# codex-storage/nim-groth16

Measured on AMD Instinct MI355X. Metric: proofs/sec (BN254 Groth16, 2^20-constraint circuit), higher is better.
Workload: dtype u32 (254-bit Montgomery: 8x32-bit limbs; 9x29-bit limbs in the bucket accumulation); 1 GPU; BN254 2^20-constraint synthetic R1CS (squaring chain, m=2^20-2), full prove: buildABC + 6 NTT + 4 G1 MSM + 1 G2 MSM, snarkjs flavour, 1 proof/step/GPU (3 proofs in flight per GPU, one shared key); mode=replica, nvars=1048576, domain_log2=20

## Files before the change

### nim_groth16_amd/csrc/msm.cuh

```cuda
#pragma once
#include "ec29.cuh"
#include "msm_params.hpp"

namespace g16 {

#ifndef G16_ACC_BLOCK
#define G16_ACC_BLOCK 256
#endif
constexpr int ACC_BLOCK = G16_ACC_BLOCK;
#ifndef G16_G2_WAVES
#define G16_G2_WAVES 2
#endif

#ifndef G16_TAIL_PRIO
#define G16_TAIL_PRIO 0
#endif
__device__ __forceinline__ void tail_prio() {
#if G16_TAIL_PRIO
  __builtin_amdgcn_s_setprio(G16_TAIL_PRIO);
#endif
}
#ifndef G16_G1_WAVES
#define G16_G1_WAVES 4
#endif
#ifndef G16_TAIL_WAVES_G1
#define G16_TAIL_WAVES_G1 1
#endif
#ifndef G16_TAIL_WAVES_G2
#define G16_TAIL_WAVES_G2 1
#endif
template <class C>
constexpr int tail_waves() { return sizeof(typename C::Aff) == 64 ? G16_TAIL_WAVES_G1 : G16_TAIL_WAVES_G2; }

constexpr int MSM_BATCH_MAX = 3;
template <class C>
struct MsmJob {
  const typename Ec29<C>::Tab* points;
  const uint32_t* entries;
  const uint32_t* offset;
  const uint2* xseg;
  const uint32_t* info;
  const uint32_t* perm;
  const uint32_t* heavy;
  const uint32_t* xoff;
  typename Ec29<C>::Acc* partial;
  const typename Ec29<C>::Acc* init;
  typename C::Acc* chunkR;
  typename C::Acc* chunkA;
  typename C::Acc* wsum;
  typename C::Aff* out_aff;
  typename C::Acc* out_acc;
};
template <class C>
struct MsmBatch {
  MsmJob<C> job[MSM_BATCH_MAX];
};



template <class EMIT>
__device__ __forceinline__ void msm_digits(const u256* __restrict__ scalars, const uint32_t* __restrict__ live, uint32_t i,
                                           const MsmParams& P, EMIT&& emit) {
  if (live && !((live[i >> 5] >> (i & 31)) & 1u)) return;
  u256 s = scalars[i];
  if (P.scalars_mont) s = Fr::from_mont(s);
  if (Fr::is_zero(s)) return;
  const uint32_t c = P.c, half = 1u << (c - 1), mask = (1u << c) - 1;
  uint32_t carry = 0;
  for (uint32_t w = 0; w < P.nwin; ++w) {
    uint32_t raw = (s.v[0] & mask) + carry;
    uint32_t neg = raw > half ? 1u : 0u;
    uint32_t mag = neg ? (1u << c) - raw : raw;
    carry = neg;
    if (mag) {
      if (P.mtab == 2) {
        uint32_t sel;
        const uint32_t b = msm_class_bucket(mag, c, sel);
        emit(w + sel * P.nwin, b, neg);
      } else {
        emit(w, mag - 1, neg);
      }
    }
#pragma unroll
    for (int j = 0; j < 7; ++j) s.v[j] = __builtin_amdgcn_alignbit(s.v[j + 1], s.v[j], c);
    s.v[7] >>= c;
  }
}

template <bool LEAN>
__device__ __forceinline__ void msm_entry_place(const MsmParams& P, uint32_t w, uint32_t i, uint32_t shift,
                                                uint32_t& set_off, uint32_t& pidx) {
  if (LEAN) {
    uint32_t table, set;
    msm_window_slot(w, P.tstride, table, set);
    set_off = set << shift;
    pidx = table * P.n + i;
  } else {
    set_off = P.tables ? 0u : (w << shift);
    pidx = P.tables ? (w * P.n + i) : i;
  }
}

template <bool LEAN>
static __global__ void __launch_bounds__(MSM_BLOCK) msm_count(const u256* __restrict__ scalars,
                                                              const uint32_t* __restrict__ live, MsmParams P,
                                                              uint32_t* __restrict__ count) {
  uint32_t i = blockIdx.x * MSM_BLOCK + threadIdx.x;
  if (i >= P.n) return;
  const uint32_t bshift = P.c - 1;
  msm_digits(scalars, live, i, P, [&](uint32_t w, uint32_t k, uint32_t) {
    uint32_t set_off, pidx;
    msm_entry_place<LEAN>(P, w, i, bshift, set_off, pidx);
    atomicAdd(&count[set_off + k], 1u);
  });
}

template <bool LEAN>
static __global__ void __launch_bounds__(MSM_BLOCK) msm_scatter(const u256* __restrict__ scalars,
                                                         const uint32_t* __restrict__ live, MsmParams P,
                                                         const uint32_t* __restrict__ offset,
                                                         uint32_t* __restrict__ cursor,
                                                         uint32_t* __restrict__ entries) {
  uint32_t i = blockIdx.x * MSM_BLOCK + threadIdx.x;
  if (i >= P.n) return;
  const uint32_t bshift = P.c - 1;
  msm_digits(scalars, live, i, P, [&](uint32_t w, uint32_t k, uint32_t neg) {
    uint32_t set_off, pidx;
    msm_entry_place<LEAN>(P, w, i, bshift, set_off, pidx);
    uint32_t b = set_off + k;
    uint32_t pos = offset[b] + atomicAdd(&cursor[b], 1u);
    entries[pos] = pidx | (neg << 31);
  });
}

__device__ __forceinline__ uint32_t lds_rank_add(uint32_t* ctr, uint32_t key) {
  const uint32_t leader = __builtin_amdgcn_readfirstlane(key);
  const unsigned long long m = __ballot(key == leader);
  if (__popcll(m) > 8) {
    uint32_t r = 0;
    if (key == leader) {
      const uint32_t lane = threadIdx.x & 63;
      const uint32_t before = __popcll(m & ((1ull << lane) - 1));
      uint32_t base = 0;
      if (before == 0) base = atomicAdd(&ctr[leader], (uint32_t)__popcll(m));
      base = __shfl(base, __ffsll((long long)m) - 1, 64);
      r = base + before;
    } else {
      r = atomicAdd(&ctr[key], 1u);
    }
    return r;
  }
  return atomicAdd(&ctr[key], 1u);
}

__device__ __forceinline__ uint32_t part_tile_of_block(uint32_t bid, uint32_t ntiles) {
  return (ntiles & 7u) ? bid : (bid & 7u) * (ntiles >> 3) + (bid >> 3);
}
template <bool SCATTER, bool LEAN>
static __global__ void __launch_bounds__(PART_BLOCK) part_pass(const u256* __restrict__ scalars,
                                                               const uint32_t* __restrict__ live, MsmParams P,
                                                               uint32_t lo_bits, uint32_t nparts, uint32_t ntiles,
                                                               uint32_t* __restrict__ tile_hist,
                                                               uint2* __restrict__ tmp) {
  __shared__ uint32_t hist[PART_MAX];
  const uint32_t tile = part_tile_of_block(blockIdx.x, ntiles);
  for (uint32_t p = threadIdx.x; p < nparts; p += PART_BLOCK)
    hist[p] = SCATTER ? tile_hist[(size_t)p * ntiles + tile] : 0u;
  __syncthreads();
  const uint32_t hi_bits = P.c - 1 - lo_bits, lo_mask = (1u << lo_bits) - 1;
  for (uint32_t r = 0; r < PART_PER_THREAD; ++r) {
    uint32_t i = tile * PART_TILE + r * PART_BLOCK + threadIdx.x;
    if (i < P.n) {
      msm_digits(scalars, live, i, P, [&](uint32_t w, uint32_t k, uint32_t neg) {
        uint32_t set_off, pidx;
        msm_entry_place<LEAN>(P, w, i, hi_bits, set_off, pidx);
        uint32_t part = set_off | (k >> lo_bits);
        uint32_t pos = lds_rank_add(hist, part);
        if (SCATTER) tmp[pos] = make_uint2((k & lo_mask) | (neg << BS_LOG), pidx);
      });
    }
  }
  if (!SCATTER) {
    __syncthreads();
    for (uint32_t p = threadIdx.x; p < nparts; p += PART_BLOCK) tile_hist[(size_t)p * ntiles + tile] = hist[p];
  }
}

__device__ __forceinline__ void bs_slice(uint32_t start, uint32_t end, uint32_t q, uint32_t& lo, uint32_t& hi) {
  const uint32_t len = end - start;
  lo = start + (uint32_t)(((uint64_t)len * q) / BS_SPLIT);
  hi = start + (uint32_t)(((uint64_t)len * (q + 1)) / BS_SPLIT);
}
static __global__ void __launch_bounds__(BS_LOW) bucket_hist(const uint2* __restrict__ tmp,
                                                          const uint32_t* __restrict__ part_base, uint32_t ntiles,
                                                          uint32_t nparts, const uint32_t* __restrict__ total,
                                                          uint32_t* __restrict__ slice_hist) {
  __shared__ uint32_t hist[BS_LOW];
  uint32_t part, q;
  bs_block(blockIdx.x, nparts, part, q);
  const uint32_t tid = threadIdx.x;
  const uint32_t start = part_base[(size_t)part * ntiles];
  const uint32_t end = part + 1 < nparts ? part_base[(size_t)(part + 1) * ntiles] : total[0];
  uint32_t lo, hi;
  bs_slice(start, end, q, lo, hi);
  hist[tid] = 0;
  __syncthreads();
  for (uint32_t j = lo + tid; j < hi; j += BS_LOW) lds_rank_add(hist, tmp[j].x & (uint32_t)(BS_LOW - 1));
  __syncthreads();
  slice_hist[((size_t)part * BS_SPLIT + q) * BS_LOW + tid] = hist[tid];
}
__device__ __forceinline__ uint32_t extra_segs(uint32_t cnt, uint32_t L) { return cnt > L ? (cnt - 1) / L : 0u; }
static __global__ void __launch_bounds__(BS_LOW) bucket_place(const uint2* __restrict__ tmp,
                                                           const uint32_t* __restrict__ part_base, uint32_t ntiles,
                                                           uint32_t nparts, const uint32_t* __restrict__ total,
                                                           const uint32_t* __restrict__ slice_hist, MsmParams P,
                                                           uint32_t lo_bits, uint32_t* __restrict__ count,
                                                           uint32_t* __restrict__ offset,
                                                           uint32_t* __restrict__ entries, uint32_t fused,
                                                           uint32_t* __restrict__ xoff, uint32_t* __restrict__ heavy,
                                                           uint32_t* __restrict__ info, uint32_t* __restrict__ ghist,
                                                           uint32_t* __restrict__ blk_base) {
  __shared__ uint32_t cur[BS_LOW];
  __shared__ uint32_t szh[PERM_BINS];
  uint32_t part, q;
  bs_block(blockIdx.x, nparts, part, q);
  const uint32_t tid = threadIdx.x;
  const uint32_t start = part_base[(size_t)part * ntiles];
  const uint32_t end = part + 1 < nparts ? part_base[(size_t)(part + 1) * ntiles] : total[0];
  uint32_t mine = 0, before = 0;
#pragma unroll
  for (int k = 0; k < BS_SPLIT; ++k) {
    uint32_t h = slice_hist[((size_t)part * BS_SPLIT + k) * BS_LOW + tid];
    mine += h;
    if ((uint32_t)k < q) before += h;
  }
  cur[tid] = mine;
  if (tid < PERM_BINS) szh[tid] = 0;
  __syncthreads();
  for (int d = 1; d < BS_LOW; d <<= 1) {
    uint32_t add = (int)tid >= d ? cur[tid - d] : 0u;
    __syncthreads();
    cur[tid] += add;
    __syncthreads();
  }
  const uint32_t excl = cur[tid] - mine;
  __syncthreads();
  cur[tid] = start + excl + before;
  if (q == 0) {
    if (tid < (1u << lo_bits)) {
      uint32_t b = (part << lo_bits) + tid;
      count[b] = mine;
      offset[b] = start + excl;
      if (fused) {
        const uint32_t e = extra_segs(mine, P.seg);
        uint32_t x0 = 0;
        if (e) {
          x0 = atomicAdd(&info[1], e);
          heavy[atomicAdd(&info[2], 1u)] = b;
        }
        xoff[b] = x0;
        atomicAdd(&szh[mine < PERM_BINS - 1 ? mine : PERM_BINS - 1], 1u);
      }
    }
    if (part == nparts - 1 && tid == 0) offset[P.nbuckets] = end;
  }
  __syncthreads();
  if (q == 0 && fused && tid < PERM_BINS) {
    const uint32_t m = szh[tid];
    blk_base[(size_t)part * PERM_BINS + tid] = m ? atomicAdd(&ghist[tid], m) : 0u;
  }
  uint32_t lo, hi;
  bs_slice(start, end, q, lo, hi);
  for (uint32_t j = lo + tid; j < hi; j += BS_LOW) {
    uint2 e = tmp[j];
    uint32_t pos = lds_rank_add(cur, e.x & (uint32_t)(BS_LOW - 1));
    entries[pos] = e.y | (((e.x >> BS_LOG) & 1u) << 31);
  }
}


constexpr uint32_t HEAVY_MIN = 12;

__device__ __forceinline__ uint2 block_excl_scan2(uint2 v, uint2* total) {
  __shared__ uint2 wsum[SCAN_BLOCK / 64];
  const uint32_t lane = threadIdx.x & 63, wave = threadIdx.x >> 6;
  uint2 inc = v;
#pragma unroll
  for (int d = 1; d < 64; d <<= 1) {
    uint32_t x = __shfl_up(inc.x, d, 64), y = __shfl_up(inc.y, d, 64);
    if (lane >= (uint32_t)d) { inc.x += x; inc.y += y; }
  }
  if (lane == 63) wsum[wave] = inc;
  __syncthreads();
  uint2 base = make_uint2(0, 0), tot = make_uint2(0, 0);
#pragma unroll
  for (int w = 0; w < SCAN_BLOCK / 64; ++w) {
    uint2 s = wsum[w];
    if ((uint32_t)w < wave) { base.x += s.x; base.y += s.y; }
    tot.x += s.x; tot.y += s.y;
  }
  __syncthreads();
  if (total) *total = tot;
  return make_uint2(base.x + inc.x - v.x, base.y + inc.y - v.y);
}

static __global__ void __launch_bounds__(SCAN_BLOCK) scan_tile_sums(const uint32_t* __restrict__ count, uint32_t nb,
                                                             uint32_t L, uint2* __restrict__ tile_sum) {
  uint32_t base = blockIdx.x * SCAN_TILE + threadIdx.x * SCAN_ITEMS;
  uint2 s = make_uint2(0, 0);
#pragma unroll
  for (int j = 0; j < SCAN_ITEMS; ++j) {
    uint32_t b = base + j;
    uint32_t cnt = b < nb ? count[b] : 0u;
    s.x += cnt;
    s.y += extra_segs(cnt, L);
  }
  uint2 tot;
  block_excl_scan2(s, &tot);
  if (threadIdx.x == 0) tile_sum[blockIdx.x] = tot;
}
static __global__ void __launch_bounds__(SCAN_BLOCK) scan_tiles(uint2* __restrict__ tile_sum, uint32_t ntiles,
                                                         uint32_t* __restrict__ info) {
  uint2 carry = make_uint2(0, 0);
  for (uint32_t base = 0; base < ntiles; base += SCAN_BLOCK) {
    uint32_t t = base + threadIdx.x;
    uint2 v = t < ntiles ? tile_sum[t] : make_uint2(0, 0);
    uint2 tot;
    uint2 ex = block_excl_scan2(v, &tot);
    if (t < ntiles) tile_sum[t] = make_uint2(ex.x + carry.x, ex.y + carry.y);
    carry.x += tot.x;
    carry.y += tot.y;
  }
  if (threadIdx.x == 0) {
    info[0] = carry.x;
    info[1] = carry.y;
  }
}
static __global__ void __launch_bounds__(SCAN_BLOCK) scan_apply(const uint32_t* __restrict__ count, uint32_t nb, uint32_t L,
                                                         const uint2* __restrict__ tile_sum,
                                                         uint32_t* __restrict__ offset, uint32_t* __restrict__ xoff,
                                                         uint32_t* __restrict__ heavy, uint32_t* __restrict__ info) {
  uint32_t base = blockIdx.x * SCAN_TILE + threadIdx.x * SCAN_ITEMS;
  uint32_t cnt[SCAN_ITEMS];
  uint2 s = make_uint2(0, 0);
#pragma unroll
  for (int j = 0; j < SCAN_ITEMS; ++j) {
    uint32_t b = base + j;
    cnt[j] = b < nb ? count[b] : 0u;
    s.x += cnt[j];
    s.y += extra_segs(cnt[j], L);
  }
  uint2 ex = block_excl_scan2(s, nullptr);
  uint2 t0 = tile_sum[blockIdx.x];
  uint32_t o = t0.x + ex.x, x = t0.y + ex.y;
#pragma unroll
  for (int j = 0; j < SCAN_ITEMS; ++j) {
    uint32_t b = base + j;
    if (b < nb) {
      offset[b] = o;
      xoff[b] = x;
      uint32_t e = extra_segs(cnt[j], L);
      if (e) heavy[atomicAdd(&info[2], 1u)] = b;
      o += cnt[j];
      x += e;
    }
  }
  if (blockIdx.x == gridDim.x - 1 && threadIdx.x == SCAN_BLOCK - 1) offset[nb] = o;
}

static __global__ void __launch_bounds__(SCAN_BLOCK) scan1_tile_sums(const uint32_t* __restrict__ v, uint32_t n,
                                                                     uint2* __restrict__ tile_sum) {
  uint32_t base = blockIdx.x * SCAN_TILE + threadIdx.x * SCAN_ITEMS;
  uint2 s = make_uint2(0, 0);
#pragma unroll
  for (int j = 0; j < SCAN_ITEMS; ++j) s.x += base + j < n ? v[base + j] : 0u;
  uint2 tot;
  block_excl_scan2(s, &tot);
  if (threadIdx.x == 0) tile_sum[blockIdx.x] = tot;
}
static __global__ void __launch_bounds__(SCAN_BLOCK) scan1_apply(uint32_t* __restrict__ v, uint32_t n,
                                                                 const uint2* __restrict__ tile_sum) {
  uint32_t base = blockIdx.x * SCAN_TILE + threadIdx.x * SCAN_ITEMS;
  uint32_t x[SCAN_ITEMS];
  uint2 s = make_uint2(0, 0);
#pragma unroll
  for (int j = 0; j < SCAN_ITEMS; ++j) {
    x[j] = base + j < n ? v[base + j] : 0u;
    s.x += x[j];
  }
  uint2 ex = block_excl_scan2(s, nullptr);
  uint32_t o = tile_sum[blockIdx.x].x + ex.x;
#pragma unroll
  for (int j = 0; j < SCAN_ITEMS; ++j) {
    if (base + j < n) v[base + j] = o;
    o += x[j];
  }
}

static __global__ void __launch_bounds__(MSM_BLOCK) msm_make_extra(const uint32_t* __restrict__ heavy,
                                                            const uint32_t* __restrict__ info,
                                                            const uint32_t* __restrict__ offset,
                                                            const uint32_t* __restrict__ xoff, uint32_t L,
                                                            uint32_t max_extra, uint2* __restrict__ xseg) {
  const uint32_t nheavy = info[2];
  for (uint32_t h = blockIdx.x; h < nheavy; h += gridDim.x) {
    uint32_t b = heavy[h];
    uint32_t cnt = offset[b + 1] - offset[b];
    uint32_t e = extra_segs(cnt, L), x0 = xoff[b];
    for (uint32_t s = threadIdx.x; s < e; s += MSM_BLOCK)
      if (x0 + s < max_extra) xseg[x0 + s] = make_uint2(b, s + 1);
  }
}

static __global__ void __launch_bounds__(PERM_BLOCK) perm_hist(const uint32_t* __restrict__ count, uint32_t nb,
                                                               uint32_t* __restrict__ ghist,
                                                               uint32_t* __restrict__ blk_base) {
  __shared__ uint32_t h[PERM_BINS];
  if (threadIdx.x < PERM_BINS) h[threadIdx.x] = 0;
  __syncthreads();
  uint32_t b = blockIdx.x * PERM_BLOCK + threadIdx.x;
  if (b < nb) {
    uint32_t c = count[b];
    atomicAdd(&h[c < PERM_BINS - 1 ? c : PERM_BINS - 1], 1u);
  }
  __syncthreads();
  if (threadIdx.x < PERM_BINS) {
    uint32_t mine = h[threadIdx.x];
    blk_base[(size_t)blockIdx.x * PERM_BINS + threadIdx.x] = mine ? atomicAdd(&ghist[threadIdx.x], mine) : 0u;
  }
}
static __global__ void __launch_bounds__(PERM_BLOCK) perm_scatter(const uint32_t* __restrict__ count, uint32_t nb,
                                                                  const uint32_t* __restrict__ ghist,
                                                                  const uint32_t* __restrict__ blk_base,
                                                                  uint32_t* __restrict__ perm) {
  __shared__ uint32_t start[PERM_BINS];
  __shared__ uint32_t cur[PERM_BINS];
  const bool bin = threadIdx.x < PERM_BINS;
  if (bin) {
    start[threadIdx.x] = ghist[threadIdx.x];
    cur[threadIdx.x] = 0;
  }
  __syncthreads();
  for (int d = 1; d < PERM_BINS; d <<= 1) {
    uint32_t add = bin && (int)threadIdx.x + d < PERM_BINS ? start[threadIdx.x + d] : 0u;
    __syncthreads();
    if (bin) start[threadIdx.x] += add;
    __syncthreads();
  }
  uint32_t incl = bin ? start[threadIdx.x] : 0u;
  __syncthreads();
  if (bin) start[threadIdx.x] = incl - ghist[threadIdx.x];
  __syncthreads();
  uint32_t b = blockIdx.x * PERM_BLOCK + threadIdx.x;
  if (b < nb) {
    uint32_t c = count[b];
    uint32_t v = c < PERM_BINS - 1 ? c : PERM_BINS - 1;
    uint32_t r = atomicAdd(&cur[v], 1u);
    perm[start[v] + blk_base[(size_t)blockIdx.x * PERM_BINS + v] + r] = b;
  }
}

template <class C>
__global__ void __launch_bounds__(ACC_BLOCK, sizeof(typename C::Aff) == 64 ? G16_G1_WAVES : G16_G2_WAVES)
msm_accum(const MsmBatch<C> B, MsmParams P, unsigned long long* __restrict__ clk) {
  using E = Ec29<C>;
  const MsmJob<C>& J = B.job[blockIdx.y];
  const typename E::Tab* __restrict__ points = J.points;
  const uint32_t* __restrict__ entries = J.entries;
  const uint32_t* __restrict__ offset = J.offset;
  unsigned long long t0 = 0, r0 = 0;
  const bool stamp = clk != nullptr && threadIdx.x == 0;
  if (stamp) t0 = __builtin_amdgcn_s_memtime(), r0 = __builtin_amdgcn_s_memrealtime();
  const uint32_t t = blockIdx.x * ACC_BLOCK + threadIdx.x;
  const uint32_t nx = J.info[1] < P.max_extra ? J.info[1] : P.max_extra;
  uint32_t b, s, slot;
  if (t < nx) {
    uint2 d = J.xseg[t];
    b = d.x;
    s = d.y;
    slot = P.nbuckets + t;
  } else {
    if (t - nx >= P.nbuckets) return;
    b = J.perm[t - nx];
    s = 0;
    slot = b;
  }
  uint32_t beg = offset[b], end = offset[b + 1];
  beg += s * P.seg;
  if (end > beg + P.seg) end = beg + P.seg;
  typename E::Acc acc = E::acc_inf();
  if (J.init != nullptr && s == 0) acc = J.init[b];
  for (uint32_t j = beg; j < end; ++j) {
    const uint32_t e = entries[j];
    E::madd(acc, points + (e & 0x7fffffffu), e >> 31);
  }
  J.partial[slot] = acc;
  if (stamp) {
    atomicAdd(&clk[0], __builtin_amdgcn_s_memtime() - t0);
    atomicAdd(&clk[1], __builtin_amdgcn_s_memrealtime() - r0);
  }
}

template <class C>
__global__ void __launch_bounds__(MSM_BLOCK) points_to29(const typename C::Aff* __restrict__ points, uint32_t n,
                                                         typename Ec29<C>::Tab* __restrict__ out) {
  uint32_t i = blockIdx.x * MSM_BLOCK + threadIdx.x;
  if (i < n) out[i] = Ec29<C>::tab_from_std(points[i]);
}

template <class C, int BLOCK>
__device__ __forceinline__ typename C::Acc block_sum(typename C::Acc v, typename C::Acc* sh) {
  sh[threadIdx.x] = v;
  __syncthreads();
#pragma unroll 1
  for (int stride = BLOCK / 2; stride > 0; stride >>= 1) {
    if ((int)threadIdx.x < stride) {
      typename C::Acc a = sh[threadIdx.x];
      C::add(a, sh[threadIdx.x + stride]);
      sh[threadIdx.x] = a;
    }
    __syncthreads();
  }
  typename C::Acc r = sh[0];
  __syncthreads();
  return r;
}

template <class C>
constexpr int heavy_block() { return sizeof(typename C::Aff) == 64 ? 256 : 128; }
template <class C>
__global__ void __launch_bounds__(heavy_block<C>(), tail_waves<C>()) msm_heavy(const MsmBatch<C> B, MsmParams P) {
  tail_prio();
  using E = Ec29<C>;
  constexpr int HEAVY_BLOCK = heavy_block<C>();
  extern __shared__ __align__(16) unsigned char smem[];
  typename E::Acc* sh = reinterpret_cast<typename E::Acc*>(smem);
  const MsmJob<C>& J = B.job[blockIdx.y];
  const uint32_t* __restrict__ heavy = J.heavy;
  const uint32_t* __restrict__ offset = J.offset;
  const uint32_t* __restrict__ xoff = J.xoff;
  typename E::Acc* __restrict__ partial = J.partial;
  const uint32_t nheavy = J.info[2];
  for (uint32_t h = blockIdx.x * HEAVY_BLOCK + threadIdx.x; h < nheavy; h += gridDim.x * HEAVY_BLOCK) {
    const uint32_t b = heavy[h];
    const uint32_t e = extra_segs(offset[b + 1] - offset[b], P.seg), x0 = xoff[b];
    if (e >= HEAVY_MIN) continue;
    typename E::Acc acc = partial[b];
    for (uint32_t k = 0; k < e; ++k) E::add(acc, partial[P.nbuckets + x0 + k]);
    partial[b] = acc;
  }
  for (uint32_t h = blockIdx.x; h < nheavy; h += gridDim.x) {
    uint32_t b = heavy[h];
    uint32_t e = extra_segs(offset[b + 1] - offset[b], P.seg), x0 = xoff[b];
    if (e < HEAVY_MIN) continue;
    typename E::Acc acc = E::acc_inf();
    for (uint32_t s = threadIdx.x; s <= e; s += HEAVY_BLOCK) {
      uint32_t idx = s == 0 ? b : P.nbuckets + x0 + s - 1;
      E::add(acc, partial[idx]);
    }
    typename E::Acc r = block_sum<E, HEAVY_BLOCK>(acc, sh);
    if (threadIdx.x == 0) partial[b] = r;
  }
}

template <class C>
__global__ void __launch_bounds__(MSM_BLOCK, tail_waves<C>()) msm_reduce1(const MsmBatch<C> B, uint32_t nbuckets, uint32_t rc) {
  tail_prio();
  using E = Ec29<C>;
  const MsmJob<C>& J = B.job[blockIdx.y];
  const typename E::Acc* __restrict__ partial = J.partial;
  const uint32_t* __restrict__ offset = J.offset;
  const bool always = J.init != nullptr;
  uint32_t j = blockIdx.x * MSM_BLOCK + threadIdx.x;
  uint32_t b0 = j * rc;
  if (b0 >= nbuckets) return;
  typename E::Acc run = E::acc_inf(), acc = E::acc_inf();
#pragma unroll 1
  for (int k = (int)rc - 1; k >= 0; --k) {
    uint32_t b = b0 + k;
    if (b < nbuckets && (always || offset[b + 1] != offset[b])) E::add(run, partial[b]);
    E::add(acc, run);
  }
  J.chunkR[j] = E::to_std(run);
  J.chunkA[j] = E::to_std(acc);
}
template <class C, int BLOCK>
__global__ void __launch_bounds__(BLOCK, tail_waves<C>()) msm_reduce2(const MsmBatch<C> B, uint32_t chunks_per_window,
                                                                      uint32_t rc) {
  tail_prio();
  extern __shared__ __align__(16) unsigned char smem[];
  typename C::Acc* sh = reinterpret_cast<typename C::Acc*>(smem);
  const MsmJob<C>& J = B.job[blockIdx.y];
  typename C::Acc* __restrict__ window_sum = J.wsum;
  typename C::Acc* __restrict__ window_tot = J.wsum + 65;
  const uint32_t w = blockIdx.x, M = chunks_per_window;
  const typename C::Acc* R = J.chunkR + (size_t)w * M;
  const typename C::Acc* A = J.chunkA + (size_t)w * M;
  const uint32_t per = (M + BLOCK - 1) / BLOCK;
  const uint32_t lo = threadIdx.x * per, hi = (lo + per < M) ? lo + per : M;
  typename C::Acc sumA = C::acc_inf(), run = C::acc_inf(), wsum = C::acc_inf();
  if (lo < M) {
    for (uint32_t m = hi; m-- > lo;) {
      C::add(wsum, run);
      C::add(run, R[m]);
      C::add(sumA, A[m]);
    }
  }
  sh[threadIdx.x] = run;
  __syncthreads();
  typename C::Acc incl = run;
#pragma unroll 1
  for (int d = 1; d < BLOCK; d <<= 1) {
    typename C::Acc other = C::acc_inf();
    const bool has = (int)threadIdx.x + d < BLOCK;
    if (has) other = sh[threadIdx.x + d];
    __syncthreads();
    if (has) C::add(incl, other);
    sh[threadIdx.x] = incl;
    __syncthreads();
  }
  if (threadIdx.x == 0) window_tot[w] = incl;
  typename C::Acc v = (threadIdx.x >= 1 && lo < M) ? C::mul_small(incl, per) : C::acc_inf();
  C::add(v, wsum);
  v = C::mul_small(v, rc);
  C::add(v, sumA);
  __syncthreads();
  typename C::Acc tot = block_sum<C, BLOCK>(v, sh);
  if (threadIdx.x == 0) window_sum[w] = tot;
}

__device__ __forceinline__ u256 wave_get(const u256& v, int src) {
  u256 r;
#pragma unroll
  for (int i = 0; i < 8; ++i) r.v[i] = __shfl(v.v[i], src, 64);
  return r;
}
__device__ __forceinline__ fp2_t wave_get(const fp2_t& v, int src) { return fp2_t{wave_get(v.c0, src), wave_get(v.c1, src)}; }
template <class E>
__device__ __forceinline__ E sel3(uint32_t role, const E& a, const E& b, const E& c) {
  return role == 0 ? a : (role == 1 ? b : c);
}
template <class C>
__device__ __forceinline__ typename C::Acc dbl_coop(const typename C::Acc& p) {
  using F = typename C::Field;
  using E = typename C::E;
  const uint32_t lane = threadIdx.x & 63, role = lane < 2 ? lane : 2;
  const E u = F::dbl(p.y);
  const E l1 = F::sqr(role == 0 ? u : p.x);
  const E v = wave_get(l1, 0), xx = wave_get(l1, 1);
  const E m = F::add(F::dbl(xx), xx);
  const E l2 = F::mul(sel3(role, u, p.x, m), role == 2 ? m : v);
  const E w = wave_get(l2, 0), s = wave_get(l2, 1), mm = wave_get(l2, 2);
  const E x3 = F::sub(mm, F::dbl(s));
  const E l3 = F::mulsub(sel3(role, m, v, w), sel3(role, F::sub(s, x3), p.zz, p.zzz), role == 0 ? w : F::zero(), p.y);
  return typename C::Acc{x3, wave_get(l3, 0), wave_get(l3, 1), wave_get(l3, 2)};
}

template <int I>
__device__ __forceinline__ uint32_t quad_word(uint32_t v) {
  return (uint32_t)__builtin_amdgcn_update_dpp(0, (int)v, I * 0x55, 0xf, 0xf, false);
}
template <int I>
__device__ __forceinline__ u256 quad_get(const u256& v) {
  u256 r;
#pragma unroll
  for (int i = 0; i < 8; ++i) r.v[i] = quad_word<I>(v.v[i]);
  return r;
}
template <int I>
__device__ __forceinline__ fp2_t quad_get(const fp2_t& v) { return fp2_t{quad_get<I>(v.c0), quad_get<I>(v.c1)}; }
template <class E>
__device__ __forceinline__ E sel4(uint32_t role, const E& a, const E& b, const E& c, const E& d) {
  return role == 0 ? a : (role == 1 ? b : (role == 2 ? c : d));
}
template <class C>
__device__ __forceinline__ typename C::Acc dbl_quad(const typename C::Acc& p) {
  using F = typename C::Field;
  using E = typename C::E;
  const uint32_t q = threadIdx.x & 3, role = q < 2 ? q : 2;
  const E u = F::dbl(p.y);
  const E l1 = F::sqr(role == 0 ? u : p.x);
  const E v = quad_get<0>(l1), xx = quad_get<1>(l1);
  const E m = F::add(F::dbl(xx), xx);
  const E l2 = F::mul(sel3(role, u, p.x, m), role == 2 ? m : v);
  const E w = quad_get<0>(l2), s = quad_get<1>(l2), mm = quad_get<2>(l2);
  const E x3 = F::sub(mm, F::dbl(s));
  const E l3 = F::mulsub(sel3(role, m, v, w), sel3(role, F::sub(s, x3), p.zz, p.zzz), role == 0 ? w : F::zero(), p.y);
  return typename C::Acc{x3, quad_get<0>(l3), quad_get<1>(l3), quad_get<2>(l3)};
}
template <class C>
__device__ __forceinline__ typename C::Acc add_quad(const typename C::Acc& a, const typename C::Acc& b) {
  using F = typename C::Field;
  using E = typename C::E;
  if (C::is_inf(b)) return a;
  if (C::is_inf(a)) return b;
  const uint32_t role = threadIdx.x & 3;
  const E l1 = F::mul(sel4(role, a.x, b.x, a.y, b.y), sel4(role, b.zz, a.zz, b.zzz, a.zzz));
  const E u1 = quad_get<0>(l1), u2 = quad_get<1>(l1), s1 = quad_get<2>(l1), s2 = quad_get<3>(l1);
  const E p = F::sub(u2, u1), r = F::sub(s2, s1);
  if (F::is_zero(p)) return F::is_zero(r) ? dbl_quad<C>(a) : C::acc_inf();
  const E l2 = F::mul(sel4(role, p, r, a.zz, a.zzz), sel4(role, p, r, b.zz, b.zzz));
  const E pp = quad_get<0>(l2), rr = quad_get<1>(l2), z12 = quad_get<2>(l2), z123 = quad_get<3>(l2);
  const E l3 = F::mul(sel4(role, p, u1, z12, z12), pp);
  const E ppp = quad_get<0>(l3), qq = quad_get<1>(l3), zz3 = quad_get<2>(l3);
  const E x3 = F::sub(F::sub(rr, ppp), F::dbl(qq));
  const E l4 = F::mul(sel4(role, r, s1, z123, z123), role == 0 ? F::sub(qq, x3) : ppp);
  return typename C::Acc{x3, F::sub(quad_get<0>(l4), quad_get<1>(l4)), zz3, quad_get<2>(l4)};
}
template <class C>
__device__ __forceinline__ typename C::Acc mul_small_quad(const typename C::Acc& p, uint32_t k) {
  typename C::Acc r = C::acc_inf();
#pragma unroll 1
  for (int b = k ? 31 - __clz(k) : -1; b >= 0; --b) {
    r = dbl_quad<C>(r);
    if ((k >> b) & 1) r = add_quad<C>(r, p);
  }
  return r;
}
template <class C, int SLOTS>
__device__ __forceinline__ typename C::Acc block_sum_quad(const typename C::Acc& v, typename C::Acc* sh) {
  const int slot = threadIdx.x >> 2;
  __syncthreads();
  if ((threadIdx.x & 3) == 0) sh[slot] = v;
  __syncthreads();
#pragma unroll 1
  for (int stride = SLOTS / 2; stride > 0; stride >>= 1) {
    if (slot < stride) {
      const typename C::Acc a = add_quad<C>(sh[slot], sh[slot + stride]);
      if ((threadIdx.x & 3) == 0) sh[slot] = a;
    }
    __syncthreads();
  }
  const typename C::Acc r = sh[0];
  __syncthreads();
// ... 324 lines not shown
```

### nim_groth16_amd/csrc/msm_params.hpp

```cpp
#pragma once
#include <stdint.h>

namespace g16 {
struct MsmParams {
  uint32_t n;
  uint32_t c;
  uint32_t nwin;
  uint32_t nbuckets;
  uint32_t seg;
  uint32_t scalars_mont;
  uint32_t tables;
  uint32_t max_extra;
  uint32_t mtab;
  uint32_t tstride = 0;
};
inline uint32_t msm_table_buckets(uint32_t c, uint32_t mtab) {
  const uint32_t h = 1u << (c - 1);
  return mtab == 2 ? h / 2 + h / 8 + h / 32 + h / 64 : h;
}
constexpr uint32_t MSM_CLASS_SLICES = 32 + 8 + 2 + 1;
#if defined(__HIPCC__)
#define G16_MSMP_HD __host__ __device__ __forceinline__
#else
#define G16_MSMP_HD inline
#endif

constexpr int MSM_BLOCK = 256;
constexpr int FR_BITS = 254;
constexpr int BS_LOG = 9;
constexpr int BS_LOW = 1 << BS_LOG;
constexpr int PART_BLOCK = 1024;
constexpr int PART_PER_THREAD = 4;
constexpr int PART_TILE = PART_BLOCK * PART_PER_THREAD;
constexpr int PART_MAX = 8192;
constexpr int PERM_BINS = 256;
constexpr int PERM_BLOCK = BS_LOW;
constexpr int SCAN_BLOCK = 256;
constexpr int SCAN_ITEMS = 8;
constexpr int SCAN_TILE = SCAN_BLOCK * SCAN_ITEMS;

constexpr int BS_SPLIT = 8;
G16_MSMP_HD void bs_block(uint32_t bid, uint32_t nparts, uint32_t& part, uint32_t& q) {
  if (BS_SPLIT == 8 && (nparts & 7u) == 0) {
    const uint32_t j = bid >> 3;
    part = ((j >> 3) << 3) | (bid & 7u);
    q = j & 7u;
  } else {
    part = bid / BS_SPLIT;
    q = bid % BS_SPLIT;
  }
}
G16_MSMP_HD void msm_window_slot(uint32_t w, uint32_t tstride, uint32_t& table, uint32_t& set) {
  if (tstride == 1) {
    table = w;
    set = 0;
  } else if (tstride == 0) {
    table = 0;
    set = w;
  } else {
    table = w / tstride;
    set = w - table * tstride;
  }
}
G16_MSMP_HD uint32_t msm_class_bucket(uint32_t t, uint32_t c, uint32_t& s) {
  const uint32_t tz = (uint32_t)__builtin_ctz(t), h = 1u << (c - 1);
  if (tz >= 6) {
    s = 0;
    return h / 2 + h / 8 + h / 32 + (t >> 6) - 1;
  }
  s = tz & 1u;
  const uint32_t z = tz >> 1, v = (t >> (tz + 1));
  const uint32_t base = z == 0 ? 0u : z == 1 ? h / 2 : h / 2 + h / 8;
  return base + v;
}
}
```

### nim_groth16_amd/csrc/msm_sort.hip

```cpp
#include "g16_internal.hpp"
#include "msm.cuh"

using namespace g16;

static_assert(MSM_FLAG_SCALARS_MONT == G16_SCALARS_MONT, "msm_plan.hpp and the C ABI disagree on the Montgomery flag");

int32_t g16_msm_sort(g16_ctx* ctx, hipStream_t st, const void* d_scalars, uint32_t flags, size_t n, uint32_t table_cfg,
                     g16_ctx::MsmSort& S, const uint32_t* d_live) {
  const G16Env& env = g16_env();
  const MsmParams P = msm_params(n, flags, table_cfg, env);
  const MsmSortPlan L = msm_sort_plan(P, env);
  S.P = P;
  Carver measure{nullptr}, bind{nullptr};
  msm_sort_layout(S, P, L, measure);
  if (int32_t rc = ensure(ctx, S.buf, measure.bytes)) return rc;
  bind.base = (char*)S.buf.p();
  msm_sort_layout(S, P, L, bind);
  const auto* scalars = (const u256*)d_scalars;
  if (!L.use_part) HIPCHK(ctx, hipMemsetAsync(S.count, 0, (char*)S.offset - (char*)S.count, st));
  HIPCHK(ctx, hipMemsetAsync(S.info, 0, 64, st));
  HIPCHK(ctx, hipMemsetAsync(S.ghist, 0, PERM_BINS * 4, st));
  const bool lean = P.tstride >= 2;
  if (L.use_part) {
    if (lean)
      KLAUNCH_ON(ctx, st, "msm_part_count", (part_pass<false, true>), L.ptiles, PART_BLOCK, 0, scalars, d_live, P, L.lo_bits,
                 L.nparts, L.ptiles, S.tile_hist, S.tmp);
    else
      KLAUNCH_ON(ctx, st, "msm_part_count", (part_pass<false, false>), L.ptiles, PART_BLOCK, 0, scalars, d_live, P, L.lo_bits,
                 L.nparts, L.ptiles, S.tile_hist, S.tmp);
    KLAUNCH_ON(ctx, st, "msm_scan", scan1_tile_sums, L.nt2, SCAN_BLOCK, 0, S.tile_hist, (uint32_t)L.nth, S.tiles2);
    KLAUNCH_ON(ctx, st, "msm_scan", scan_tiles, 1, SCAN_BLOCK, 0, S.tiles2, L.nt2, S.info + 8);
    KLAUNCH_ON(ctx, st, "msm_scan", scan1_apply, L.nt2, SCAN_BLOCK, 0, S.tile_hist, (uint32_t)L.nth, S.tiles2);
    if (lean)
      KLAUNCH_ON(ctx, st, "msm_part_scatter", (part_pass<true, true>), L.ptiles, PART_BLOCK, 0, scalars, d_live, P, L.lo_bits,
                 L.nparts, L.ptiles, S.tile_hist, S.tmp);
    else
      KLAUNCH_ON(ctx, st, "msm_part_scatter", (part_pass<true, false>), L.ptiles, PART_BLOCK, 0, scalars, d_live, P, L.lo_bits,
                 L.nparts, L.ptiles, S.tile_hist, S.tmp);
    KLAUNCH_ON(ctx, st, "msm_bucket_sort", bucket_hist, L.nparts * BS_SPLIT, BS_LOW, 0, S.tmp, S.tile_hist, L.ptiles,
               L.nparts, S.info + 8, S.slice_hist);
    KLAUNCH_ON(ctx, st, "msm_bucket_sort", bucket_place, L.nparts * BS_SPLIT, BS_LOW, 0, S.tmp, S.tile_hist, L.ptiles,
               L.nparts, S.info + 8, S.slice_hist, P, L.lo_bits, S.count, S.offset, S.entries, L.fused ? 1u : 0u, S.xoff,
               S.heavy, S.info, S.ghist, S.blk_base);
  } else {
    if (lean)
      KLAUNCH_ON(ctx, st, "msm_count", msm_count<true>, L.nblk, MSM_BLOCK, 0, scalars, d_live, P, S.count);
    else
      KLAUNCH_ON(ctx, st, "msm_count", msm_count<false>, L.nblk, MSM_BLOCK, 0, scalars, d_live, P, S.count);
  }
  if (!L.fused) {
    KLAUNCH_ON(ctx, st, "msm_scan", scan_tile_sums, L.ntiles, SCAN_BLOCK, 0, S.count, P.nbuckets, P.seg, S.tiles);
    KLAUNCH_ON(ctx, st, "msm_scan", scan_tiles, 1, SCAN_BLOCK, 0, S.tiles, L.ntiles, S.info);
    KLAUNCH_ON(ctx, st, "msm_scan", scan_apply, L.ntiles, SCAN_BLOCK, 0, S.count, P.nbuckets, P.seg, S.tiles, S.offset,
               S.xoff, S.heavy, S.info);
    KLAUNCH_ON(ctx, st, "msm_perm", perm_hist, L.pblk, PERM_BLOCK, 0, S.count, P.nbuckets, S.ghist, S.blk_base);
  }
  KLAUNCH_ON(ctx, st, "msm_perm", perm_scatter, L.pblk, PERM_BLOCK, 0, S.count, P.nbuckets, S.ghist, S.blk_base,
             S.perm);
  if (!L.use_part) {
    if (lean)
      KLAUNCH_ON(ctx, st, "msm_scatter", msm_scatter<true>, L.nblk, MSM_BLOCK, 0, scalars, d_live, P, S.offset, S.cursor,
                 S.entries);
    else
      KLAUNCH_ON(ctx, st, "msm_scatter", msm_scatter<false>, L.nblk, MSM_BLOCK, 0, scalars, d_live, P, S.offset, S.cursor,
                 S.entries);
  }
  KLAUNCH_ON(ctx, st, "msm_make_extra", msm_make_extra, 512, MSM_BLOCK, 0, S.heavy, S.info, S.offset, S.xoff, P.seg,
             P.max_extra, S.xseg);
  HIPCHK(ctx, hipGetLastError());
  return G16_OK;
}

template <class C>
static int32_t msm_batch(g16_ctx* ctx, hipStream_t st, const g16_msm_run* runs, int n_accum, int n_tail,
                         hipEvent_t after_heavy) {
  if (n_accum < 1 || n_accum > MSM_BATCH_MAX || n_tail < 0 || n_tail > n_accum) {
    ctx->err = "bad MSM batch";
    return G16_EINVAL;
  }
  const MsmParams& P = runs[0].sort->P;
  constexpr size_t asz = sizeof(typename C::Acc);
  constexpr size_t psz29 = sizeof(typename Ec29<C>::Acc);
  static_assert(asz == 2 * sizeof(typename C::Aff) && psz29 * 8 == asz * 9, "accumulator sizes");
  const MsmTailPlan T = msm_tail_plan(P, sizeof(typename C::Aff) == 64, runs[0].sort->narrow_tail, g16_env());
  MsmBatch<C> B;
  memset(&B, 0, sizeof B);
  Carver measure{nullptr};
  msm_job_layout(B.job[0], P, T.nchunks, asz, psz29, measure);
  for (int j = 0; j < n_accum; ++j) {
    const g16_ctx::MsmSort& S = *runs[j].sort;
    const MsmParams& Q = S.P;
    if (Q.n != P.n || Q.c != P.c || Q.nwin != P.nwin || Q.nbuckets != P.nbuckets || Q.seg != P.seg ||
        Q.tables != P.tables || Q.mtab != P.mtab || Q.tstride != P.tstride || Q.max_extra != P.max_extra) {
      ctx->err = "MSM batch: the jobs do not share their launch parameters";
      return G16_EINVAL;
    }
    if (int32_t rc = ensure(ctx, *runs[j].acc, measure.bytes)) return rc;
    MsmJob<C>& J = B.job[j];
    Carver bind{(char*)runs[j].acc->p()};
    msm_job_layout(J, P, T.nchunks, asz, psz29, bind);
    J.points = (const typename Ec29<C>::Tab*)runs[j].d_points;
    J.entries = S.entries;
    J.offset = S.offset;
    J.xseg = S.xseg;
    J.info = S.info;
    J.perm = S.perm;
    J.heavy = S.heavy;
    J.xoff = S.xoff;
    J.init = (const typename Ec29<C>::Acc*)runs[j].init_partial;
    J.out_aff = (typename C::Aff*)runs[j].d_out_aff;
    J.out_acc = (typename C::Acc*)runs[j].d_out_acc;
  }
  int32_t rc;
  if ((rc = stage_accum<C>(ctx, st, P, B, n_accum))) return rc;
  if ((rc = stage_heavy<C>(ctx, st, P, T, B, n_accum))) return rc;
  if (after_heavy) HIPCHK(ctx, hipEventRecord(after_heavy, st));
  if (!n_tail) return G16_OK;
  if ((rc = stage_reduce1<C>(ctx, st, P, T, B, n_tail))) return rc;
  return stage_reduce2_fold<C>(ctx, st, P, T, B, n_tail);
}
int32_t g16_msm_batch(g16_ctx* ctx, hipStream_t stream, int group, const g16_msm_run* runs, int n_accum, int n_tail,
                      hipEvent_t after_heavy) {
  return group == 1 ? msm_batch<G1>(ctx, stream, runs, n_accum, n_tail, after_heavy)
                    : msm_batch<G2>(ctx, stream, runs, n_accum, n_tail, after_heavy);
}

template <class C>
int32_t msm_device(g16_ctx* ctx, const void* d_scalars, uint32_t flags, const void* d_points, size_t n, void* d_out_aff,
                   void* d_out_acc, uint32_t table_c, const uint32_t* d_live) {
  ctx->sort[0].narrow_tail = false;
  int32_t rc = g16_msm_sort(ctx, ctx->stream, d_scalars, flags, n, table_c, ctx->sort[0], d_live);
  if (rc) return rc;
  if ((table_c & 0xffu) == 0 && n) {
    static_assert(sizeof(typename Ec29<C>::Tab) == sizeof(typename C::Aff), "packed entries: 64 / 128 B");
    if ((rc = ensure(ctx, ctx->stage_p29, n * sizeof(typename Ec29<C>::Tab)))) return rc;
    if ((rc = to29_device<C>(ctx, ctx->stream, d_points, n, ctx->stage_p29.p()))) return rc;
    d_points = ctx->stage_p29.p();
  }
  const g16_msm_run run{&ctx->sort[0], &ctx->lane[0].acc, d_points, d_out_aff, d_out_acc, nullptr};
  return msm_batch<C>(ctx, ctx->stream, &run, 1, 1, nullptr);
}
template int32_t msm_device<G1>(g16_ctx*, const void*, uint32_t, const void*, size_t, void*, void*, uint32_t, const uint32_t*);
template int32_t msm_device<G2>(g16_ctx*, const void*, uint32_t, const void*, size_t, void*, void*, uint32_t, const uint32_t*);
```

Baseline: 117.9 proofs/s.

## Cap front-end sort kernels' VGPRs to co-reside with G1 accumulation waves

Introduces a VGPR budget for the MSM sort/scan/partition kernels so they fit in the register space left over when four G1 accumulation waves (120 VGPRs each) occupy a SIMD. This lets the sort of one in-flight proof overlap with another proof's bucket accumulation. It also shrinks the partition block from 1024 to 256 threads while raising per-thread items to 16, moves the partition histogram to dynamic LDS, and disables unrolling in a few loops to reduce register pressure. Tight VGPR caps may cause spills in the front kernels, and smaller partition blocks change tile counts.

Result: no change. 117.7 proofs/s (-0.2%).

```diff
diff --git a/nim_groth16_amd/csrc/msm.cuh b/nim_groth16_amd/csrc/msm.cuh
--- a/nim_groth16_amd/csrc/msm.cuh
+++ b/nim_groth16_amd/csrc/msm.cuh
@@ -29,6 +29,8 @@
 #ifndef G16_TAIL_WAVES_G2
 #define G16_TAIL_WAVES_G2 1
 #endif
+#define G16_FRONT_KERNEL(threads, budget) \
+  __launch_bounds__(threads) __attribute__((amdgpu_num_vgpr(front_vgprs(threads, budget) / 2)))
 template <class C>
 constexpr int tail_waves() { return sizeof(typename C::Aff) == 64 ? G16_TAIL_WAVES_G1 : G16_TAIL_WAVES_G2; }
 
@@ -102,7 +104,7 @@
 }
 
 template <bool LEAN>
-static __global__ void __launch_bounds__(MSM_BLOCK) msm_count(const u256* __restrict__ scalars,
+static __global__ void G16_FRONT_KERNEL(MSM_BLOCK, FRONT_VGPRS) msm_count(const u256* __restrict__ scalars,
                                                               const uint32_t* __restrict__ live, MsmParams P,
                                                               uint32_t* __restrict__ count) {
   uint32_t i = blockIdx.x * MSM_BLOCK + threadIdx.x;
@@ -116,7 +118,7 @@
 }
 
 template <bool LEAN>
-static __global__ void __launch_bounds__(MSM_BLOCK) msm_scatter(const u256* __restrict__ scalars,
+static __global__ void G16_FRONT_KERNEL(MSM_BLOCK, FRONT_VGPRS) msm_scatter(const u256* __restrict__ scalars,
                                                          const uint32_t* __restrict__ live, MsmParams P,
                                                          const uint32_t* __restrict__ offset,
                                                          uint32_t* __restrict__ cursor,
@@ -157,17 +159,18 @@
   return (ntiles & 7u) ? bid : (bid & 7u) * (ntiles >> 3) + (bid >> 3);
 }
 template <bool SCATTER, bool LEAN>
-static __global__ void __launch_bounds__(PART_BLOCK) part_pass(const u256* __restrict__ scalars,
+static __global__ void G16_FRONT_KERNEL(PART_BLOCK, FRONT_VGPRS) part_pass(const u256* __restrict__ scalars,
                                                                const uint32_t* __restrict__ live, MsmParams P,
                                                                uint32_t lo_bits, uint32_t nparts, uint32_t ntiles,
                                                                uint32_t* __restrict__ tile_hist,
                                                                uint2* __restrict__ tmp) {
-  __shared__ uint32_t hist[PART_MAX];
+  extern __shared__ uint32_t hist[];
   const uint32_t tile = part_tile_of_block(blockIdx.x, ntiles);
   for (uint32_t p = threadIdx.x; p < nparts; p += PART_BLOCK)
     hist[p] = SCATTER ? tile_hist[(size_t)p * ntiles + tile] : 0u;
   __syncthreads();
   const uint32_t hi_bits = P.c - 1 - lo_bits, lo_mask = (1u << lo_bits) - 1;
+#pragma unroll 1
   for (uint32_t r = 0; r < PART_PER_THREAD; ++r) {
     uint32_t i = tile * PART_TILE + r * PART_BLOCK + threadIdx.x;
     if (i < P.n) {
@@ -191,7 +194,7 @@
   lo = start + (uint32_t)(((uint64_t)len * q) / BS_SPLIT);
   hi = start + (uint32_t)(((uint64_t)len * (q + 1)) / BS_SPLIT);
 }
-static __global__ void __launch_bounds__(BS_LOW) bucket_hist(const uint2* __restrict__ tmp,
+static __global__ void G16_FRONT_KERNEL(BS_LOW, FRONT_VGPRS) bucket_hist(const uint2* __restrict__ tmp,
                                                           const uint32_t* __restrict__ part_base, uint32_t ntiles,
                                                           uint32_t nparts, const uint32_t* __restrict__ total,
                                                           uint32_t* __restrict__ slice_hist) {
@@ -210,7 +213,7 @@
   slice_hist[((size_t)part * BS_SPLIT + q) * BS_LOW + tid] = hist[tid];
 }
 __device__ __forceinline__ uint32_t extra_segs(uint32_t cnt, uint32_t L) { return cnt > L ? (cnt - 1) / L : 0u; }
-static __global__ void __launch_bounds__(BS_LOW) bucket_place(const uint2* __restrict__ tmp,
+static __global__ void G16_FRONT_KERNEL(BS_LOW, FRONT_VGPRS) bucket_place(const uint2* __restrict__ tmp,
                                                            const uint32_t* __restrict__ part_base, uint32_t ntiles,
                                                            uint32_t nparts, const uint32_t* __restrict__ total,
                                                            const uint32_t* __restrict__ slice_hist, MsmParams P,
@@ -304,7 +307,7 @@
   return make_uint2(base.x + inc.x - v.x, base.y + inc.y - v.y);
 }
 
-static __global__ void __launch_bounds__(SCAN_BLOCK) scan_tile_sums(const uint32_t* __restrict__ count, uint32_t nb,
+static __global__ void G16_FRONT_KERNEL(SCAN_BLOCK, FRONT_VGPRS_MIXED) scan_tile_sums(const uint32_t* __restrict__ count, uint32_t nb,
                                                              uint32_t L, uint2* __restrict__ tile_sum) {
   uint32_t base = blockIdx.x * SCAN_TILE + threadIdx.x * SCAN_ITEMS;
   uint2 s = make_uint2(0, 0);
@@ -319,7 +322,7 @@
   block_excl_scan2(s, &tot);
   if (threadIdx.x == 0) tile_sum[blockIdx.x] = tot;
 }
-static __global__ void __launch_bounds__(SCAN_BLOCK) scan_tiles(uint2* __restrict__ tile_sum, uint32_t ntiles,
+static __global__ void G16_FRONT_KERNEL(SCAN_BLOCK, FRONT_VGPRS) scan_tiles(uint2* __restrict__ tile_sum, uint32_t ntiles,
                                                          uint32_t* __restrict__ info) {
   uint2 carry = make_uint2(0, 0);
   for (uint32_t base = 0; base < ntiles; base += SCAN_BLOCK) {
@@ -336,39 +339,39 @@
     info[1] = carry.y;
   }
 }
-static __global__ void __launch_bounds__(SCAN_BLOCK) scan_apply(const uint32_t* __restrict__ count, uint32_t nb, uint32_t L,
+static __global__ void G16_FRONT_KERNEL(SCAN_BLOCK, FRONT_VGPRS_MIXED) scan_apply(const uint32_t* __restrict__ count, uint32_t nb, uint32_t L,
                                                          const uint2* __restrict__ tile_sum,
                                                          uint32_t* __restrict__ offset, uint32_t* __restrict__ xoff,
                                                          uint32_t* __restrict__ heavy, uint32_t* __restrict__ info) {
   uint32_t base = blockIdx.x * SCAN_TILE + threadIdx.x * SCAN_ITEMS;
-  uint32_t cnt[SCAN_ITEMS];
   uint2 s = make_uint2(0, 0);
 #pragma unroll
   for (int j = 0; j < SCAN_ITEMS; ++j) {
     uint32_t b = base + j;
-    cnt[j] = b < nb ? count[b] : 0u;
-    s.x += cnt[j];
-    s.y += extra_segs(cnt[j], L);
+    uint32_t cnt = b < nb ? count[b] : 0u;
+    s.x += cnt;
+    s.y += extra_segs(cnt, L);
   }
   uint2 ex = block_excl_scan2(s, nullptr);
   uint2 t0 = tile_sum[blockIdx.x];
   uint32_t o = t0.x + ex.x, x = t0.y + ex.y;
-#pragma unroll
+#pragma unroll 1
   for (int j = 0; j < SCAN_ITEMS; ++j) {
     uint32_t b = base + j;
     if (b < nb) {
+      const uint32_t cnt = count[b];
       offset[b] = o;
       xoff[b] = x;
-      uint32_t e = extra_segs(cnt[j], L);
+      uint32_t e = extra_segs(cnt, L);
       if (e) heavy[atomicAdd(&info[2], 1u)] = b;
-      o += cnt[j];
+      o += cnt;
       x += e;
     }
   }
   if (blockIdx.x == gridDim.x - 1 && threadIdx.x == SCAN_BLOCK - 1) offset[nb] = o;
 }
 
-static __global__ void __launch_bounds__(SCAN_BLOCK) scan1_tile_sums(const uint32_t* __restrict__ v, uint32_t n,
+static __global__ void G16_FRONT_KERNEL(SCAN_BLOCK, FRONT_VGPRS_MIXED) scan1_tile_sums(const uint32_t* __restrict__ v, uint32_t n,
                                                                      uint2* __restrict__ tile_sum) {
   uint32_t base = blockIdx.x * SCAN_TILE + threadIdx.x * SCAN_ITEMS;
   uint2 s = make_uint2(0, 0);
@@ -378,7 +381,7 @@
   block_excl_scan2(s, &tot);
   if (threadIdx.x == 0) tile_sum[blockIdx.x] = tot;
 }
-static __global__ void __launch_bounds__(SCAN_BLOCK) scan1_apply(uint32_t* __restrict__ v, uint32_t n,
+static __global__ void G16_FRONT_KERNEL(SCAN_BLOCK, FRONT_VGPRS_MIXED) scan1_apply(uint32_t* __restrict__ v, uint32_t n,
                                                                  const uint2* __restrict__ tile_sum) {
   uint32_t base = blockIdx.x * SCAN_TILE + threadIdx.x * SCAN_ITEMS;
   uint32_t x[SCAN_ITEMS];
@@ -397,7 +400,7 @@
   }
 }
 
-static __global__ void __launch_bounds__(MSM_BLOCK) msm_make_extra(const uint32_t* __restrict__ heavy,
+static __global__ void G16_FRONT_KERNEL(MSM_BLOCK, FRONT_VGPRS_MIXED) msm_make_extra(const uint32_t* __restrict__ heavy,
                                                             const uint32_t* __restrict__ info,
                                                             const uint32_t* __restrict__ offset,
                                                             const uint32_t* __restrict__ xoff, uint32_t L,
@@ -412,7 +415,7 @@
   }
 }
 
-static __global__ void __launch_bounds__(PERM_BLOCK) perm_hist(const uint32_t* __restrict__ count, uint32_t nb,
+static __global__ void G16_FRONT_KERNEL(PERM_BLOCK, FRONT_VGPRS) perm_hist(const uint32_t* __restrict__ count, uint32_t nb,
                                                                uint32_t* __restrict__ ghist,
                                                                uint32_t* __restrict__ blk_base) {
   __shared__ uint32_t h[PERM_BINS];
@@ -429,7 +432,7 @@
     blk_base[(size_t)blockIdx.x * PERM_BINS + threadIdx.x] = mine ? atomicAdd(&ghist[threadIdx.x], mine) : 0u;
   }
 }
-static __global__ void __launch_bounds__(PERM_BLOCK) perm_scatter(const uint32_t* __restrict__ count, uint32_t nb,
+static __global__ void G16_FRONT_KERNEL(PERM_BLOCK, FRONT_VGPRS) perm_scatter(const uint32_t* __restrict__ count, uint32_t nb,
                                                                   const uint32_t* __restrict__ ghist,
                                                                   const uint32_t* __restrict__ blk_base,
                                                                   uint32_t* __restrict__ perm) {
diff --git a/nim_groth16_amd/csrc/msm_params.hpp b/nim_groth16_amd/csrc/msm_params.hpp
--- a/nim_groth16_amd/csrc/msm_params.hpp
+++ b/nim_groth16_amd/csrc/msm_params.hpp
@@ -27,12 +27,26 @@
 
 constexpr int MSM_BLOCK = 256;
 constexpr int FR_BITS = 254;
+constexpr int SIMD_VGPRS = 512;
+constexpr int VGPR_GRANULE = 8;
+constexpr int ACCUM_G1_WAVES = 4;
+constexpr int ACCUM_G1_VGPRS_ALLOC = 120;
+constexpr int FRONT_VGPRS = SIMD_VGPRS - ACCUM_G1_WAVES * ACCUM_G1_VGPRS_ALLOC;
+constexpr int FRONT_VGPRS_MIXED = 24;
+constexpr int FRONT_WAVES_PER_SIMD = 1;
+constexpr int FRONT_BLOCK = 256 * FRONT_WAVES_PER_SIMD;
+static_assert(FRONT_VGPRS == 32 && FRONT_VGPRS % VGPR_GRANULE == 0 && FRONT_VGPRS_MIXED % VGPR_GRANULE == 0, "front budget");
+constexpr int front_vgprs(int threads, int budget = FRONT_VGPRS) {
+  return budget / ((threads + 255) / 256) / VGPR_GRANULE * VGPR_GRANULE;
+}
+
 constexpr int BS_LOG = 9;
 constexpr int BS_LOW = 1 << BS_LOG;
-constexpr int PART_BLOCK = 1024;
-constexpr int PART_PER_THREAD = 4;
+constexpr int PART_BLOCK = FRONT_BLOCK;
+constexpr int PART_PER_THREAD = 16;
 constexpr int PART_TILE = PART_BLOCK * PART_PER_THREAD;
 constexpr int PART_MAX = 8192;
+constexpr int PART_LDS_BYTES = PART_MAX * 4;
 constexpr int PERM_BINS = 256;
 constexpr int PERM_BLOCK = BS_LOW;
 constexpr int SCAN_BLOCK = 256;
diff --git a/nim_groth16_amd/csrc/msm_sort.hip b/nim_groth16_amd/csrc/msm_sort.hip
--- a/nim_groth16_amd/csrc/msm_sort.hip
+++ b/nim_groth16_amd/csrc/msm_sort.hip
@@ -23,19 +23,19 @@
   const bool lean = P.tstride >= 2;
   if (L.use_part) {
     if (lean)
-      KLAUNCH_ON(ctx, st, "msm_part_count", (part_pass<false, true>), L.ptiles, PART_BLOCK, 0, scalars, d_live, P, L.lo_bits,
+      KLAUNCH_ON(ctx, st, "msm_part_count", (part_pass<false, true>), L.ptiles, PART_BLOCK, PART_LDS_BYTES, scalars, d_live, P, L.lo_bits,
                  L.nparts, L.ptiles, S.tile_hist, S.tmp);
     else
-      KLAUNCH_ON(ctx, st, "msm_part_count", (part_pass<false, false>), L.ptiles, PART_BLOCK, 0, scalars, d_live, P, L.lo_bits,
+      KLAUNCH_ON(ctx, st, "msm_part_count", (part_pass<false, false>), L.ptiles, PART_BLOCK, PART_LDS_BYTES, scalars, d_live, P, L.lo_bits,
                  L.nparts, L.ptiles, S.tile_hist, S.tmp);
     KLAUNCH_ON(ctx, st, "msm_scan", scan1_tile_sums, L.nt2, SCAN_BLOCK, 0, S.tile_hist, (uint32_t)L.nth, S.tiles2);
     KLAUNCH_ON(ctx, st, "msm_scan", scan_tiles, 1, SCAN_BLOCK, 0, S.tiles2, L.nt2, S.info + 8);
     KLAUNCH_ON(ctx, st, "msm_scan", scan1_apply, L.nt2, SCAN_BLOCK, 0, S.tile_hist, (uint32_t)L.nth, S.tiles2);
     if (lean)
-      KLAUNCH_ON(ctx, st, "msm_part_scatter", (part_pass<true, true>), L.ptiles, PART_BLOCK, 0, scalars, d_live, P, L.lo_bits,
+      KLAUNCH_ON(ctx, st, "msm_part_scatter", (part_pass<true, true>), L.ptiles, PART_BLOCK, PART_LDS_BYTES, scalars, d_live, P, L.lo_bits,
                  L.nparts, L.ptiles, S.tile_hist, S.tmp);
     else
-      KLAUNCH_ON(ctx, st, "msm_part_scatter", (part_pass<true, false>), L.ptiles, PART_BLOCK, 0, scalars, d_live, P, L.lo_bits,
+      KLAUNCH_ON(ctx, st, "msm_part_scatter", (part_pass<true, false>), L.ptiles, PART_BLOCK, PART_LDS_BYTES, scalars, d_live, P, L.lo_bits,
                  L.nparts, L.ptiles, S.tile_hist, S.tmp);
     KLAUNCH_ON(ctx, st, "msm_bucket_sort", bucket_hist, L.nparts * BS_SPLIT, BS_LOW, 0, S.tmp, S.tile_hist, L.ptiles,
                L.nparts, S.info + 8, S.slice_hist);
```
